# Codeuser0717/CVAE-GAN

Measured on NVIDIA B200. Metric: train_samples_per_s, higher is better.
Workload: dtype f32

## Files before the change

cvae_gan_b200/csrc/api.cu:

```cuda
#include "engine.cuh"

namespace cvg {
const char* last_error();
int comm_unique_id(void* out128);
int comm_init(Engine& e, const void* id128, int rank, int world);
void comm_destroy(Engine& e);
}

using namespace cvg;

struct CvgHandle {
  Engine e;
};

#define H_OR_FAIL(h)                      \
  if (!(h)) {                             \
    cvg::set_error("null handle");        \
    return 1;                             \
  }


constexpr int FC_MAX_KC = 12;
template <int KC>
struct FcDispatch {
// ... 34 lines not shown
int cvg_abi_version(void) { return CVG_ABI_VERSION; }
int cvg_config_bytes(void) { return (int)sizeof(CvgConfig); }

int cvg_create(const CvgConfig* cfg, CvgHandle** out) {
  if (!cfg || !out) CVG_FAIL("cvg_create: null argument");
  *out = nullptr;
  int dev = 0;
  CVG_CUDA(cudaGetDevice(&dev));
  cudaDeviceProp prop;
  CVG_CUDA(cudaGetDeviceProperties(&prop, dev));
  if (prop.major != 10)
    CVG_FAIL(std::string("cvaegan_b200 runs on sm_100 (B200) only; device is sm_") + std::to_string(prop.major) +
             std::to_string(prop.minor) + " - there is no fallback path");
  if (cfg->feature_num < 1 || cfg->label_num < 1 || cfg->z_size < 4 || cfg->max_batch < 1)
    CVG_FAIL("cvg_create: bad dimensions");
  if (cfg->world_size < 1 || cfg->rank < 0 || cfg->rank >= cfg->world_size) CVG_FAIL("cvg_create: bad rank/world_size");
  CvgHandle* h = new CvgHandle();
  Engine& e = h->e;
  e.cfg = *cfg;
  e.F = cfg->feature_num;
  e.K = cfg->label_num;
  e.Kc = cfg->unconditional ? 0 : cfg->label_num;
  e.Z = cfg->z_size;
  e.world = cfg->world_size;
  e.rank = cfg->rank;
  e.num_sms = prop.multiProcessorCount;
  if (build_layouts(e) != 0) {
    delete h;
    return 1;
  }
  set_all_kernel_attributes();
  tc_set_kernel_attributes();
  {
    const char* off = getenv("CVG_DISABLE_TC");
    e.use_tc = tc_supported(e) && !(off && off[0] == '1');
    const char* tm = getenv("CVG_TRAIN_MODE");
    e.mk.enabled = mk_supported(e) && tm && !strcmp(tm, "mk");
    if (const char* hv = getenv("CVG_HOIST")) e.hoist = atoi(hv) != 0;
    const char* coop = getenv("CVG_MK_COOP");
    e.mk.coop = !(coop && coop[0] == '0');
    const char* ab = getenv("CVG_MK_ALLBAR");
    e.mk.allbar = ab && ab[0] == '1';
  }
  if (cudaGetLastError() != cudaSuccess) {
    cvg::set_error("cudaFuncSetAttribute failed");
    delete h;
    return 1;
  }
  {
    SideStreams& ms = h->e.ms;
    const char* off = getenv("CVG_STREAMS");
    ms.on = !(off && off[0] == '0');
    bool ok = true;
    for (int i = 0; i < 2 && ok; ++i) ok = cudaStreamCreateWithFlags(&ms.s[i], cudaStreamNonBlocking) == cudaSuccess;
    for (int i = 0; i < SIDE_EVENTS && ok; ++i) ok = cudaEventCreateWithFlags(&ms.ev[i], cudaEventDisableTiming) == cudaSuccess;
    for (int i = 0; i < 4 && ok; ++i) ok = cudaEventCreateWithFlags(&ms.layer[i], cudaEventDisableTiming) == cudaSuccess;
    if (!ok) {
      cvg::set_error("creating the side streams failed");
      cvg_destroy(h);
      return 1;
    }
  }
  *out = h;
  return 0;
}

void cvg_destroy(CvgHandle* h) {
  if (!h) return;
  for (int i = 0; i < 2; ++i)
    if (h->e.ms.s[i]) cudaStreamDestroy(h->e.ms.s[i]);
  for (int i = 0; i < SIDE_EVENTS; ++i)
    if (h->e.ms.ev[i]) cudaEventDestroy(h->e.ms.ev[i]);
  for (int i = 0; i < 4; ++i)
    if (h->e.ms.layer[i]) cudaEventDestroy(h->e.ms.layer[i]);
  nvl_destroy(h->e);
  comm_destroy(h->e);
  mk_destroy(h->e);
  delete h;
}

int cvg_net_sizes(const CvgHandle* h, int net, int64_t* n_param_floats, int64_t* n_state_floats) {
  H_OR_FAIL(h);
  if (net < 0 || net >= CVG_NUM_NETS) CVG_FAIL("bad net id");
  if (n_param_floats) *n_param_floats = h->e.lay[net].n_param;
  if (n_state_floats) *n_state_floats = h->e.lay[net].n_state;
  return 0;
}

int cvg_tensor_table(const CvgHandle* h, int net, CvgTensorDesc* out, int32_t capacity, int32_t* count) {
  H_OR_FAIL(h);
  if (net < 0 || net >= CVG_NUM_NETS) CVG_FAIL("bad net id");
  const auto& t = h->e.lay[net].table;
  if (count) *count = (int32_t)t.size();
  if (out) {
    if (capacity < (int32_t)t.size()) CVG_FAIL("tensor table capacity too small");
    for (size_t i = 0; i < t.size(); ++i) out[i] = t[i];
  }
  return 0;
}

int64_t cvg_workspace_bytes(const CvgHandle* h) { return h ? workspace_bytes(h->e) : -1; }

int cvg_bind_net(CvgHandle* h, int net, float* params, float* grads, float* adam_m, float* adam_v, float* state) {
  H_OR_FAIL(h);
  if (net < 0 || net >= CVG_NUM_NETS) CVG_FAIL("bad net id");
  if (!params || !grads || !adam_m || !adam_v) CVG_FAIL("cvg_bind_net: null buffer");
  if (h->e.lay[net].n_state > 0 && !state) CVG_FAIL("cvg_bind_net: this network needs a state buffer");
  if ((((uintptr_t)params | (uintptr_t)grads | (uintptr_t)adam_m | (uintptr_t)adam_v | (uintptr_t)state) & 15) != 0)
    CVG_FAIL("cvg_bind_net: buffers must be 16-byte aligned");
  NetBuffers& b = h->e.buf[net];
  b.params = params; b.grads = grads; b.m = adam_m; b.v = adam_v; b.state = state;
  return 0;
}

int cvg_bind_workspace(CvgHandle* h, void* workspace, int64_t bytes, void* stream) {
  H_OR_FAIL(h);
  if (!workspace) CVG_FAIL("null workspace");
  CVG_TRY(carve_workspace(h->e, workspace, bytes));
  if (mk_supported(h->e)) CVG_TRY(mk_alloc_slots(h->e));
  CVG_CUDA(cudaMemsetAsync(workspace, 0, (size_t)bytes, (cudaStream_t)stream));
  return 0;
}
// ... 262 lines not shown
int cvg_debug_tc_counters(CvgHandle* h, long long* dev_counters) {
  H_OR_FAIL(h);
  h->e.tc_dbg = dev_counters;
  return 0;
}

int cvg_profile_enable(CvgHandle* h, int enable) {
  H_OR_FAIL(h);
  Engine& e = h->e;
  for (auto& r : e.prof_recs) {
    cudaEventDestroy(r.a);
    cudaEventDestroy(r.b);
  }
  e.prof_recs.clear();
  e.prof = enable != 0;
  return 0;
}

int cvg_profile_read(CvgHandle* h, int kernel_class, int64_t* launches, double* flops, double* ms) {
  H_OR_FAIL(h);
  if (!launches || !flops || !ms) CVG_FAIL("cvg_profile_read: null argument");
  Engine& e = h->e;
  *launches = 0;
  *flops = 0.0;
  *ms = 0.0;
  for (auto& r : e.prof_recs) {
    if (r.cls != kernel_class) continue;
    CVG_CUDA(cudaEventSynchronize(r.b));
    float t = 0.f;
    CVG_CUDA(cudaEventElapsedTime(&t, r.a, r.b));
    *launches += 1;
    *flops += r.flops;
    *ms += (double)t;
  }
  return 0;
}

int64_t cvg_launch_count(const CvgHandle* h) { return h ? h->e.launches : -1; }

int cvg_debug_set(CvgHandle* h, const char* key, int value) {
  H_OR_FAIL(h);
  if (!key) CVG_FAIL("null key");
  Engine& e = h->e;
  const std::string k(key);
  if (k == "train_mode") {
    if (value && !mk_supported(e)) CVG_FAIL("cvg_debug_set: the step-program kernel does not cover these layer widths");
    e.mk.enabled = value != 0;
  } else if (k == "mk_max_ops") e.mk.max_ops = value;
  else if (k == "mk_allbar") e.mk.allbar = value != 0;
  else if (k == "mk_coop") e.mk.coop = value != 0;
  else if (k == "hoist") e.hoist = value != 0;
  else if (k == "streams") e.ms.on = value != 0;
  else if (k == "chain") e.chain = value != 0;
  else if (k == "fuse_stats") e.nvl.fuse = value != 0;
  else CVG_FAIL("cvg_debug_set: unknown key");
  return 0;
}

int cvg_debug_get(const CvgHandle* h, const char* key, int* value) {
  H_OR_FAIL(h);
  if (!key || !value) CVG_FAIL("null argument");
  const Engine& e = h->e;
  const std::string k(key);
  if (k == "train_mode") *value = e.mk.enabled ? 1 : 0;
  else if (k == "mk_last_nops") *value = e.mk.last_nops;
  else if (k == "mk_supported") *value = mk_supported(e) ? 1 : 0;
  else CVG_FAIL("cvg_debug_get: unknown key");
  return 0;
}

int cvg_debug_mk_cycles(CvgHandle* h, long long* out, int capacity, int* count) {
  H_OR_FAIL(h);
  Engine& e = h->e;
  if (!e.ws_base) CVG_FAIL("workspace not bound");
  const int n = e.mk.last_nops < capacity ? e.mk.last_nops : capacity;
  if (count) *count = n;
  if (out && n > 0) CVG_CUDA(cudaMemcpy(out, e.ws.mk_dbg, sizeof(long long) * n, cudaMemcpyDeviceToHost));
  if (out && capacity >= 2048 + 64 && n <= 1024) {
    CVG_CUDA(cudaMemcpy(out + 1024, e.ws.mk_dbg + 1024, sizeof(long long) * n, cudaMemcpyDeviceToHost));
    if (capacity >= 4096)
      for (int i = 0; i < n && i < (int)e.mk.last_kinds.size(); ++i) out[3072 + i] = e.mk.last_kinds[i];
  }
  if (out && capacity >= 2048 + 64) CVG_CUDA(cudaMemcpy(out + 2048, e.ws.mk_dbg + 2048, sizeof(long long) * 64, cudaMemcpyDeviceToHost));
  return 0;
}

}
```

cvae_gan_b200/csrc/engine.cuh:

```cuda
#pragma once
#include "common.cuh"
#include "gemm.cuh"
#include "misc_kernels.cuh"
#include "comm_nvl.cuh"

typedef struct ncclComm* ncclComm_t;

namespace cvg {

constexpr int HOIST_MAX = 16;
constexpr int STAT_C = 1024;

constexpr int DET_MAX_PASS = 4;

struct Workspace {
  int ld = 0;
  int rows_cap = 0;
  float* xT = nullptr;
  float* z = nullptr;
  uint8_t* d_m1 = nullptr;
  uint8_t* d_m2 = nullptr;
  uint8_t* c_m1 = nullptr;
  uint8_t* c_m2 = nullptr;
  float *g_h[3] = {nullptr, nullptr, nullptr};
  float* g_out = nullptr;
  float* hz = nullptr;
  float* hh[3] = {nullptr, nullptr, nullptr};
  float* hout = nullptr;
  double* hfst = nullptr;
  float *g_dy[3] = {nullptr, nullptr, nullptr};
  float* g_dout = nullptr;
  float *e_h[3] = {nullptr, nullptr, nullptr};
  float* e_ml = nullptr;
  float *e_dy[3] = {nullptr, nullptr, nullptr};
  float* e_dml = nullptr;
  float *d_a[3] = {nullptr, nullptr, nullptr};
  float* d_s = nullptr;
  float *d_g[3] = {nullptr, nullptr, nullptr};
  float* c_a1 = nullptr;
  float* c_h2 = nullptr;
  float* c_a2 = nullptr;
  float* c_rs = nullptr;
  float* c_a3 = nullptr;
  float* c_logit = nullptr;
  float* c_dlogit = nullptr;
  float *c_g[3] = {nullptr, nullptr, nullptr};
  float* dx = nullptr;
  float* sn_sigma = nullptr;
  float* sn_inv_sigma = nullptr;
  float* sn_u = nullptr;
  float* sn_v = nullptr;
  long long sn_snap = 0;
  float* sn_G = nullptr;
  double* acc = nullptr;
  size_t acc_bytes = 0;
  double* loss = nullptr;
  double* g_fst = nullptr;
  double* g_bst = nullptr;
  double* e_fst = nullptr;
  double* e_bst = nullptr;
  unsigned long long* gen_count = nullptr;
  StepCtl* ctl = nullptr;
  float* x_stage = nullptr;
  float* tc_w = nullptr;
  float* tc_c = nullptr;
  float* dw_scratch = nullptr;
  long long dw_scratch_floats = 0;
  unsigned long long* det_acc[3] = {};
  unsigned* det_cnt[3] = {};
  long long det_acc_n = 0;
  int det_cnt_n = 0;
  unsigned int* mk_bar = nullptr;
  float* z_eps = nullptr;
  float* mk_wprep = nullptr;
  long long mk_wprep_floats = 0;
  long long* mk_dbg = nullptr;
};

struct MkSlot {
  void* dev = nullptr;
  void* host = nullptr;
  size_t bytes = 0;
  unsigned long long hash = 0;
  cudaEvent_t ev = nullptr;
  bool in_graph = false;
  unsigned long long last_use = 0;
};
struct MkPrepSlot {
  const float* W = nullptr;
  int ldw = 0, wcol0 = 0, wt = 0, R = 0, N = 0, net = -1;
  long long off = 0;
  bool fresh = false;
};
struct MkPendingRed {
  unsigned char bytes[160];
  int items;
};
struct MkState {
  bool enabled = true;
  bool coop = true;
  bool allbar = false;
  int max_ops = -1;
  bool recording = false;
  bool par_next = false;
  std::vector<unsigned char> ops;
  int nops = 0;
  int phase_items = 0;
  long long scratch_off = 0;
  int n_exchanges = 0;
  int adam_inc[4] = {0, 0, 0, 0};
  unsigned long long dcounter = 0;
  std::vector<MkPendingRed> pending_red;
  std::vector<MkPrepSlot> prep;
  long long prep_off = 0;
  bool prep_open = false;
  const float* src_rows = nullptr;
  long long src_n = 0, src_Bg = 0, src_off = 0;
  std::vector<MkSlot> slots;
  unsigned long long clock = 0;
  int last_nops = 0;
  std::vector<int> last_kinds;
};

struct ProfRec {
  cudaEvent_t a, b;
  int cls;
  double flops;
};

constexpr int SIDE_EVENTS = 32;
struct SideStreams {
  bool on = false;
  cudaStream_t s[2] = {nullptr, nullptr};
  cudaEvent_t ev[SIDE_EVENTS] = {};
  cudaEvent_t layer[4] = {};
  unsigned next = 0;
  bool dirty[2] = {false, false};
};

struct Engine {
  bool prof = false;
  std::vector<ProfRec> prof_recs;
  CvgConfig cfg{};
  int F = 0, K = 0, Z = 0;
  int Kc = 0;
  int eh[3]{}, gh[3]{}, dh[3]{}, ch[3]{};
  NetLayout lay[4];
  NetBuffers buf[4];
  Workspace ws;
  void* ws_base = nullptr;
  int64_t ws_bytes = 0;
  int64_t launches = 0;
  const float* hoist_x = nullptr;
  SideStreams ms;
  bool in_visit = false;
  unsigned long long step_dcounter = 0;
  int hoist = 1;
  bool chain = true;
  ncclComm_t comm = nullptr;
  int world = 1, rank = 0;
  NvlState nvl;
  int num_sms = 148;
  long long* tc_dbg = nullptr;
  bool use_tc = true;
  MkState mk;

  float* P(int net, int64_t off) const { return buf[net].params + off; }
  float* G(int net, int64_t off) const { return buf[net].grads + off; }
  float* S(int net, int64_t off) const { return buf[net].state + off; }
};

struct CvgHandleImpl {
  Engine e;
};

int build_layouts(Engine& e);
int64_t workspace_bytes(const Engine& e);
int carve_workspace(Engine& e, void* base, int64_t bytes);

struct StepRng {
  bool set = true;
  uint64_t seed = 0, counter = 0, off = 0;
  float lambda_class = 0.f;
  bool lambda_nonzero = true;
};
int step_d(Engine& e, const float* x_real, int label, int B, const CvgNoise* noise, const StepRng& rng, int flags,
           float* loss_out, cudaStream_t st);
int step_c(Engine& e, const float* x_real, int label, int B, const CvgNoise* noise, const StepRng& rng, int flags,
           float* loss_out, cudaStream_t st);
int step_g(Engine& e, const float* x_real, int label, int B, const CvgNoise* noise, const StepRng& rng, int flags,
           float* loss_out, cudaStream_t st);
int visit(Engine& e, int label, int B, int64_t B_global, const float* class_rows, int64_t n_rows, const float* x_batches,
          int d_loop, int c_loop, int g_loop, int flags, float* loss_out, cudaStream_t st);
void set_all_kernel_attributes();
struct AdamOverride {
  float lr, beta1, beta2, eps;
};
int run_adam(Engine& e, int net_mask, cudaStream_t st, const AdamOverride* ov = nullptr, bool steps_advanced = false);
int step_classifier(Engine& e, const float* x, const long long* labels, int B, const CvgNoise* noise, const StepRng& rng,
                    const AdamOverride& ov, int flags, float* loss_out, cudaStream_t st);
int nvl_local_handle(Engine& e, void* out64);
int nvl_attach(Engine& e, const void* handles);
void nvl_destroy(Engine& e);
int comm_all_reduce_f32(Engine& e, float* p, int64_t n, cudaStream_t st, int channel = 0);
int comm_all_reduce_f64(Engine& e, double* p, int64_t n, cudaStream_t st);
int comm_all_reduce_stats(Engine& e, double* p, int npass, int C, cudaStream_t st);

bool mk_supported(const Engine& e);
void mk_set_kernel_attributes();
void mk_destroy(Engine& e);
int mk_alloc_slots(Engine& e);
// ... 50 lines not shown
```

cvae_gan_b200/csrc/layout.cu:

```cuda
#include "engine.cuh"

namespace cvg {

static thread_local std::string g_err;
void set_error(const std::string& msg) { g_err = msg; }
const char* last_error() { return g_err.c_str(); }

static int64_t pad4(int64_t n) { return (n + 3) & ~(int64_t)3; }

struct Builder {
  NetLayout& L;
  int64_t po = 0, so = 0;
  explicit Builder(NetLayout& l) : L(l) {}
  int64_t add(const std::string& key, int kind, int64_t d0, int64_t d1) {
    CvgTensorDesc t;
    memset(&t, 0, sizeof(t));
    snprintf(t.key, sizeof(t.key), "%s", key.c_str());
    t.kind = kind;
    t.ndim = d1 > 0 ? 2 : 1;
    t.shape[0] = d0;
    t.shape[1] = d1 > 0 ? d1 : 0;
    const int64_t n = d0 * (d1 > 0 ? d1 : 1);
    int64_t& o = kind == 0 ? po : so;
    t.offset = o;
// ... 176 lines not shown
  w.c_a3 = c.take<float>(2 * e.ch[2] * ld);
  w.c_logit = c.take<float>(2 * K * ld);
  w.c_dlogit = c.take<float>(2 * K * ld);
  w.dx = c.take<float>(F * ld);
  w.sn_sigma = c.take<float>(8);
  w.sn_inv_sigma = c.take<float>(8);
  long long snap = 0;
  for (int i = 0; i < 4; ++i) {
    const LinearP& p = e.lay[CVG_NET_DISCRIMINATOR].lin[i];
    snap += pad4(p.out > p.in ? p.out : p.in);
  }
  w.sn_snap = snap;
  w.sn_u = c.take<float>(2 * snap);
  w.sn_v = c.take<float>(2 * snap);
  w.sn_G = c.take<float>(2 * e.lay[CVG_NET_DISCRIMINATOR].n_param);
  const size_t n_acc = 16 + (size_t)(3 * 2 + 3 * 2 + 3 + 3) * 2 * STAT_C;
  w.acc = c.take<double>(n_acc);
  w.acc_bytes = n_acc * sizeof(double);
  if (w.acc) {
    w.loss = w.acc;
    w.g_fst = w.acc + 16;
    w.g_bst = w.g_fst + (size_t)3 * 2 * 2 * STAT_C;
    w.e_fst = w.g_bst + (size_t)3 * 2 * 2 * STAT_C;
    w.e_bst = w.e_fst + (size_t)3 * 2 * STAT_C;
  }
  w.gen_count = c.take<unsigned long long>(4);
  w.ctl = c.take<StepCtl>(1);
  w.x_stage = c.take<float>((size_t)rows * F);
  w.tc_w = c.take<float>((size_t)tc_prep_floats(e));
  w.tc_c = c.take<float>((size_t)tc_const_floats());
  {
    long long per = 0;
    for (int net = 0; net < 4; ++net) {
      long long t = 0;
      for (int i = 0; i < e.lay[net].nlin; ++i) {
        const LinearP& p = e.lay[net].lin[i];
        t += (long long)p.out * (((p.in + 15) & ~15) + 1);
      }
      per += t * (net == CVG_NET_GENERATOR || net == CVG_NET_DISCRIMINATOR ? 2 : 1);
    }
    w.dw_scratch_floats = 32 * per;
  }
  w.dw_scratch = c.take<float>((size_t)w.dw_scratch_floats);
  {
    int tiles = 1, cmax = 1;
    for (int net = 0; net < 4; ++net)
      for (int i = 0; i < e.lay[net].nlin; ++i) {
        const LinearP& p = e.lay[net].lin[i];
        tiles = std::max(tiles, ((p.in + 63) / 64) * ((p.out + 63) / 64));
        cmax = std::max(cmax, std::max(p.in, p.out));
      }
    w.det_acc_n = std::max((long long)tiles * DET_MAX_PASS * DW_PART, 2LL * cmax);
    w.det_cnt_n = tiles;
    for (int i = 0; i < 3; ++i) {
      w.det_acc[i] = c.take<unsigned long long>((size_t)w.det_acc_n);
      w.det_cnt[i] = c.take<unsigned>((size_t)w.det_cnt_n);
    }
  }
  {
    long long chunks = 0;
    for (int net = 0; net < 4; ++net)
      for (int i = 0; i < e.lay[net].nlin; ++i) {
        const LinearP& p = e.lay[net].lin[i];
        chunks += (long long)((p.out + 127) / 128) * ((p.in + 31) / 32) + (long long)((p.in + 127) / 128) * ((p.out + 31) / 32);
      }
    w.mk_wprep_floats = chunks * 8192;
  }
  w.mk_wprep = c.take<float>((size_t)w.mk_wprep_floats);
  w.mk_bar = c.take<unsigned int>(64);
  w.z_eps = c.take<float>((size_t)Z * ld);
  w.mk_dbg = c.take<long long>(2048 + 64);
  w.hz = c.take<float>((size_t)HOIST_MAX * Z * ld);
  for (int i = 0; i < 3; ++i) w.hh[i] = c.take<float>((size_t)HOIST_MAX * e.gh[i] * ld);
  w.hout = c.take<float>((size_t)HOIST_MAX * F * ld);
  w.hfst = c.take<double>((size_t)3 * HOIST_MAX * 2 * STAT_C);
  return c.off + 256;
}

int64_t workspace_bytes(const Engine& e) {
  Workspace tmp;
  return (int64_t)carve(e, tmp, nullptr);
}

int carve_workspace(Engine& e, void* base, int64_t bytes) {
  if ((int64_t)workspace_bytes(e) > bytes) CVG_FAIL("workspace too small");
  if (((uintptr_t)base & 255) != 0) CVG_FAIL("workspace must be 256-byte aligned");
  carve(e, e.ws, base);
  e.ws_base = base;
  e.ws_bytes = bytes;
  return 0;
}

}
```

cvae_gan_b200/csrc/train.cu:

```cuda
#include <dlfcn.h>
#include <math.h>

#include "chain.cuh"
#include "engine.cuh"
#include "mega.cuh"

namespace cvg {

#define CVG_PAR(e) do { (e).mk.par_next = true; } while (0)

struct Id128 {
  char b[128];
};
struct NcclApi {
  int (*GetUniqueId)(void*) = nullptr;
  int (*CommInitRank)(ncclComm_t*, int, Id128, int) = nullptr;
  int (*AllReduce)(const void*, void*, size_t, int, int, ncclComm_t, cudaStream_t) = nullptr;
  int (*CommDestroy)(ncclComm_t) = nullptr;
  const char* (*GetErrorString)(int) = nullptr;
  bool ok = false;
};
static NcclApi g_nccl;

static int load_nccl() {
// ... 170 lines not shown
  cudaEventRecord(r.a, st);
  e.prof_recs.push_back(r);
}
static void prof_end(Engine& e, cudaStream_t st) {
  if (!e.prof) return;
  cudaEventRecord(e.prof_recs.back().b, st);
}

static const NvlDev* take_pending(Engine& e, Operand& o) {
  if (!e.nvl.n_pending || (o.kind != OP_BN_ACT && o.kind != OP_BN_BWD)) return nullptr;
  for (int i = 0; i < e.nvl.n_pending; ++i) {
    const NvlPending pd = e.nvl.pending[i];
    int which = 0;
    if (pd.stats == o.bn.fstats + (long long)pd.pass0 * o.bn.sf) which = 1;
    if (o.kind == OP_BN_BWD && pd.stats == o.bn.bstats + (long long)pd.pass0 * o.bn.sb) which = 2;
    if (!which) continue;
    o.bn.poll = which | (pd.npass << 4) | (pd.pass0 << 12) | (e.nvl.via_lead ? 1 << 20 : 0);
    e.nvl.pending[i] = e.nvl.pending[--e.nvl.n_pending];
    return e.nvl.dev_d[pd.channel];
  }
  return nullptr;
}

int launch_mn(Engine& e, bool wt, const GemmArgs& g_in, cudaStream_t st) {
  GemmArgs g = g_in;
  if (!e.mk.recording)
    if (const NvlDev* ch = take_pending(e, g.a)) g.nvl = ch;
  const int zp = g.only_pass >= 0 ? 1 : g.npass;
  if (e.mk.recording) {
    const int nmt = (g.N + 127) / 128;
    int Nt = 64;
    if ((long long)((g.M + 63) / 64) * nmt * zp > 3 * e.num_sms / 2) Nt = 128;
    if (const char* f = getenv("CVG_MK_NT")) { if (atoi(f) == 128 && g.M > 64) Nt = 128; if (atoi(f) == 64) Nt = 64; }
    const int items = zp * nmt * ((g.M + Nt - 1) / Nt);
    const bool par = e.mk.par_next;
    const float* wp = nullptr;
    bool prepped_now = false;
    CVG_TRY(mk_weight_operand(e, g, wt, &wp, &prepped_now));
    e.mk.par_next = par && !prepped_now;
    return mk_push(e, mk::K_MN, &g, GEMM_ARGS_OP_BYTES, items, wt ? 1 : 0, Nt, 0, 0, &wp, sizeof(wp));
  }
  dim3 grid((g.M + TBM - 1) / TBM, (g.N + TBN - 1) / TBN, zp);
  const size_t smem = gemm_mn_smem(g);
  prof_begin(e, wt ? 0 : 1, 2.0 * g.M * (double)g.N * g.R * zp, st);
  const cudaError_t err = dispatch_mn(wt, g, grid, smem, st);
  prof_end(e, st);
  if (err != cudaSuccess)
    CVG_FAIL(std::string("gemm_mn launch (a.kind ") + std::to_string(g.a.kind) + ", ekind " + std::to_string(g.ekind) +
             "): " + cudaGetErrorString(err));
  e.launches++;
  return 0;
}

static int det_slot(const Engine& e, cudaStream_t st) { return st == e.ms.s[0] ? 1 : st == e.ms.s[1] ? 2 : 0; }

int launch_dw(Engine& e, const DwArgs& g0, cudaStream_t st) {
  if (e.mk.recording) return mk_push_dw(e, g0);
  DwArgs g = g0;
  const int kt = (g.K + 63) / 64, nt = (g.N + 63) / 64;
  const int target = 2 * e.num_sms;
  int nsplit = (target + kt * nt * g.npass - 1) / (kt * nt * g.npass);
  const int max_split = (g.M + DW_MC - 1) / DW_MC;
  if (nsplit > max_split) nsplit = max_split;
  if (nsplit < 1) nsplit = 1;
  int rows = (g.M + nsplit - 1) / nsplit;
  rows = ((rows + DW_MC - 1) / DW_MC) * DW_MC;
  nsplit = (g.M + rows - 1) / rows;
  g.rows_per_cta = rows;
  if (const NvlDev* ch = take_pending(e, g.p)) g.nvl = ch;
  if (const NvlDev* ch = take_pending(e, g.q)) g.nvl = ch;
  dim3 grid(kt, nt, g.npass * nsplit);
  if ((long long)kt * nt * g.npass * DW_PART > e.ws.det_acc_n || kt * nt > e.ws.det_cnt_n)
    CVG_FAIL("internal: weight-gradient launch exceeds the deterministic-reduction slots");
  const int slot = det_slot(e, st);
  prof_begin(e, 2, 2.0 * g.M * (double)g.N * g.K * g.npass, st);
  const cudaError_t err = dispatch_dw(g, nsplit, e.ws.det_acc[slot], e.ws.det_cnt[slot], grid, gemm_dw_smem(g), st);
  prof_end(e, st);
  if (err != cudaSuccess)
    CVG_FAIL(std::string("gemm_dw launch (p.kind ") + std::to_string(g.p.kind) + ", q.kind " + std::to_string(g.q.kind) +
             "): " + cudaGetErrorString(err));
  e.launches++;
  return 0;
}

static const LinearP& lin(const Engine& e, int net, int l) { return e.lay[net].lin[l]; }

static const float* label_column(const Engine& e, int net, const LinearP& p, int in_width, int label) {
  return e.Kc > 0 ? e.P(net, p.w) + in_width + label : nullptr;
}
static int label_col_index(const Engine& e, int in_width, int label) { return e.Kc > 0 ? in_width + label : -1; }

static double* fst_of(const Engine& e, int net, int l) {
  return net == CVG_NET_GENERATOR ? e.ws.g_fst + (size_t)l * 2 * 2 * STAT_C : e.ws.e_fst + (size_t)l * 2 * STAT_C;
}
static double* bst_of(const Engine& e, int net, int l) {
  return net == CVG_NET_GENERATOR ? e.ws.g_bst + (size_t)l * 2 * 2 * STAT_C : e.ws.e_bst + (size_t)l * 2 * STAT_C;
}

static BnRef bn_ref(const Engine& e, int net, int l, bool eval, bool update) {
  const LinearP& p = lin(e, net, l);
  BnRef b;
  b.fstats = fst_of(e, net, l);
  b.sf = 2 * STAT_C;
  b.bstats = bst_of(e, net, l);
  b.sb = 2 * STAT_C;
  b.gamma = e.P(net, p.gamma);
  b.beta = e.P(net, p.beta);
// ... 13 lines not shown
  g.Bg = Bg_bn;
  g.bn_eps = e.cfg.bn_eps;
  g.momentum = e.cfg.bn_momentum;
  g.slope = e.cfg.lrelu_slope;
  return g;
}

static DwArgs base_dw(const Engine& e, int M, float Bg_bn, int npass) {
  DwArgs g;
  g.M = M;
  g.ld = e.ws.ld;
  g.npass = npass;
  g.Bg = Bg_bn;
  g.bn_eps = e.cfg.bn_eps;
  g.slope = e.cfg.lrelu_slope;
  return g;
}

static int sync_stats(Engine& e, double* p, int npass, int C, bool local_bn, cudaStream_t st) {
  if (e.world <= 1 || local_bn) return 0;
  return comm_all_reduce_stats(e, p, npass, C, st);
}

static bool fold_stats(const Engine& e, bool local_bn) {
  return e.world > 1 && !local_bn && e.nvl.on && e.nvl.fuse && e.nvl.dev_d[0] && !e.mk.recording;
}
static int launch_mn_stats(Engine& e, bool wt, GemmArgs& g, int npass_sync, bool local_bn, cudaStream_t st, int channel = 0) {
  const bool fold = fold_stats(e, local_bn);
  if (!fold && channel != 0 && e.world > 1 && !local_bn) CVG_FAIL("internal: an exchange launch on a side stream");
  if (fold) { g.push = 1; g.nvl = e.nvl.dev_d[channel]; }
  CVG_TRY(launch_mn(e, wt, g, st));
  if (!fold) return sync_stats(e, g.ostats, npass_sync, g.N, local_bn, st);
  if (e.nvl.n_pending >= 8) CVG_FAIL("internal: too many folded exchanges in flight");
  const int p0 = g.only_pass > 0 ? g.only_pass : 0;
  e.nvl.pending[e.nvl.n_pending++] = NvlPending{g.ostats + (long long)p0 * g.sostats, g.only_pass >= 0 ? 1 : g.npass, p0, channel};
  return 0;
}

static cudaStream_t fork_to(Engine& e, int i, cudaStream_t st) {
  if (!e.ms.on || e.mk.recording) return st;
  cudaEvent_t ev = e.ms.ev[e.ms.next++ % SIDE_EVENTS];
  cudaEventRecord(ev, st);
  cudaStreamWaitEvent(e.ms.s[i], ev, 0);
  e.ms.dirty[i] = true;
  return e.ms.s[i];
}
static void wait_for(Engine& e, cudaStream_t waiter, cudaStream_t signaller) {
  if (waiter == signaller) return;
  cudaEvent_t ev = e.ms.ev[e.ms.next++ % SIDE_EVENTS];
  cudaEventRecord(ev, signaller);
  cudaStreamWaitEvent(waiter, ev, 0);
}
static void join_sides(Engine& e, cudaStream_t st, int only = -1) {
  for (int i = 0; i < 2; ++i) {
    if (!e.ms.dirty[i] || (only >= 0 && only != i)) continue;
    cudaEvent_t ev = e.ms.ev[e.ms.next++ % SIDE_EVENTS];
    cudaEventRecord(ev, e.ms.s[i]);
    cudaStreamWaitEvent(st, ev, 0);
    e.ms.dirty[i] = false;
  }
}

static int launch_fill(Engine& e, FillArgs& a, cudaStream_t st) {
  if (a.njobs == 0) return 0;
  if (e.mk.recording) return mk_push(e, mk::K_FILL, &a, sizeof(a), a.njobs * mk::FILL_VB);
  long long mx = 0;
  for (int i = 0; i < a.njobs; ++i) {
    long long t = (long long)a.job[i].npass * ((a.job[i].nfeat + 3) / 4) * a.M;
    if (t > mx) mx = t;
  }
  int blocks = (int)((mx + 255) / 256);
  if (blocks > 4 * e.num_sms) blocks = 4 * e.num_sms;
  if (blocks < 1) blocks = 1;
  fill_noise_kernel<<<dim3(blocks, a.njobs), 256, 0, st>>>(a);
  CVG_LAUNCH_CHECK();
  return 0;
}

static void add_job(FillArgs& a, void* out, const void* inj, int kind, int nfeat, int npass, int stream) {
  FillJob& j = a.job[a.njobs++];
  j.out = out;
  j.injected = inj;
  j.kind = kind;
  j.nfeat = nfeat;
  j.npass = npass;
  j.stream = stream;
  j.cstep = 0;
}

static int emit_zero(Engine& e, void* p, size_t bytes, cudaStream_t st) {
  if (e.mk.recording) {
    mk::ZeroArgs a;
    a.p = p; a.bytes = (long long)bytes;
    const int items = (int)((bytes / 16 + mk::THREADS * 8 - 1) / (mk::THREADS * 8));
    return mk_push(e, mk::K_ZERO, &a, sizeof(a), items < 1 ? 1 : items);
  }
  CVG_CUDA(cudaMemsetAsync(p, 0, bytes, st));
  return 0;
}

static int stage_x(Engine& e, const float* x_real, int M, cudaStream_t st) {
  if (e.mk.recording) {
    const MkState& src = e.mk;
    mk::StageArgs a;
    memset(&a, 0, sizeof(a));
    a.src = src.src_rows ? src.src_rows : x_real;
    a.n_rows = src.src_rows ? src.src_n : 0;
// ... 436 lines not shown
    g.W = e.P(net, p.w);
    g.ldw = p.in;
    if (l == 0) {
      g.ekind = EP_STORE;
      g.Y = w.dx;
      g.accumulate = dx_accumulate ? 1 : 0;
    } else {
      g.ekind = EP_DACT;
      g.act = ACT_RELU;
      g.sprev = (long long)p.in * ld;
      g.sY = (long long)p.in * ld;
      g.Y = w.c_g[l - 1];
      if (l == 3) g.prev = w.c_a3;
      if (l == 2) { g.prev = w.c_a2; g.mask = w.c_m2; g.smask = (long long)p.in * ld; g.keep_inv = keep_inv; }
      if (l == 1) { g.prev = w.c_a1; g.mask = w.c_m1; g.smask = (long long)p.in * ld; g.keep_inv = keep_inv; }
    }
    if (want_dw) CVG_PAR(e);
    CVG_TRY(launch_mn(e, false, g, st));
    if (l == 2) {
      const LinearP& p1 = lin(e, net, 1);
      LnBwdArgs a;
      a.M = M; a.ld = w.ld; a.C = p1.out; a.npass = npass;
      a.dn = w.c_g[1]; a.sdn = (long long)p1.out * ld;
      a.h = w.c_h2; a.sh = (long long)p1.out * ld;
      a.rs = w.c_rs; a.srs = 2 * (long long)ld;
      a.g = e.P(net, p1.gamma);
      a.dg = want_dw ? e.G(net, p1.gamma) : nullptr;
      a.db = want_dw ? e.G(net, p1.beta) : nullptr;
      if (e.mk.recording) {
        CVG_TRY(mk_push(e, mk::K_LN_BWD, &a, sizeof(a), npass * ((M + 31) / 32)));
      } else {
        const int slot = det_slot(e, st);
        if (2LL * a.C > e.ws.det_acc_n) CVG_FAIL("internal: LayerNorm backward exceeds the deterministic-reduction slots");
        launch_ln_bwd(a, e.ws.det_acc[slot], e.ws.det_cnt[slot], st);
        CVG_LAUNCH_CHECK();
      }
    }
  }
  return 0;
}

struct BnNetBwd {
  int net, npass;
  float* const* h;
  float* const* dy;
  const float* top_dy;
  long long s_top;
  Operand first_in;
  int first_K;
  int label_col;
  bool want_first_dx;
};

static int bwd_bn_net(Engine& e, const BnNetBwd& b, int M, float Bg_bn, float kl_coef, bool local_bn, cudaStream_t st) {
  const Workspace& w = e.ws;
  const size_t ld = w.ld;
  const int net = b.net;
  for (int l = 3; l >= 0; --l) {
    const LinearP& p = lin(e, net, l);
    Operand dy;
    if (l == 3) {
      dy.kind = OP_PLAIN; dy.rows = p.out; dy.p = b.top_dy; dy.sp = b.s_top;
    } else {
      dy.kind = OP_BN_BWD; dy.rows = p.out;
      dy.p = b.dy[l]; dy.sp = (long long)p.out * ld;
      dy.h = b.h[l]; dy.sh = (long long)p.out * ld;
      dy.bn = bn_ref(e, net, l, false, false);
    }
    if (l > 0) {
      const LinearP& pp = lin(e, net, l - 1);
      GemmArgs g = base_args(e, M, Bg_bn, b.npass);
      g.R = p.out;
      g.N = p.in;
      g.a = dy;
      g.W = e.P(net, p.w);
      g.ldw = p.in;
      g.ekind = EP_DBN;
      g.prev = b.h[l - 1];
      g.sprev = (long long)pp.out * ld;
      g.prev_bn = bn_ref(e, net, l - 1, false, false);
      g.Y = b.dy[l - 1];
      g.sY = (long long)pp.out * ld;
      g.ostats = bst_of(e, net, l - 1);
      g.sostats = 2 * STAT_C;
      CVG_TRY(launch_mn_stats(e, false, g, b.npass, local_bn, st));
    } else if (b.want_first_dx) {
      GemmArgs g = base_args(e, M, Bg_bn, b.npass);
      g.only_pass = 0;
      g.R = p.out;
      g.N = e.Z;
      g.a = dy;
      g.W = e.P(net, p.w);
      g.ldw = p.in;
      g.ekind = EP_REPARAM_BWD;
      g.mu = w.e_ml;
      g.lv = w.e_ml + (size_t)e.Z * ld;
      g.eps = e.mk.recording ? w.z_eps : w.z;
      g.kl_coef = kl_coef;
      g.Y = w.e_dml;
      CVG_TRY(launch_mn(e, false, g, st));
    }
    if (l > 0 || b.want_first_dx) CVG_PAR(e);
    DwArgs d = base_dw(e, M, Bg_bn, b.npass);
    d.N = p.out;
    d.p = dy;
    if (l == 0) {
      d.K = b.first_K;
      d.q = b.first_in;
      d.label_col = b.label_col;
    } else {
      d.K = p.in;
      d.q.kind = OP_BN_ACT;
      d.q.rows = p.in;
      d.q.p = b.h[l - 1];
      d.q.sp = (long long)p.in * ld;
      d.q.bn = bn_ref(e, net, l - 1, false, false);
    }
    d.dW = e.G(net, p.w);
    d.sdW = 0;
    d.ldw = p.in;
    d.db = e.G(net, p.b);
    if (l < 3) {
      d.dgamma = e.G(net, p.gamma);
      d.dbeta = e.G(net, p.beta);
      d.add_affine = (e.world <= 1 || local_bn || e.rank == 0) ? 1 : 0;
    }
    CVG_TRY(launch_dw(e, d, fork_to(e, 0, st)));
  }
  return 0;
}

static float net_lr(const Engine& e, int net) {
  if (net == CVG_NET_DISCRIMINATOR) return e.cfg.d_lr;
  if (net == CVG_NET_CLASSIFIER) return e.cfg.c_lr;
  return e.cfg.g_lr;
}

int run_adam(Engine& e, int net_mask, cudaStream_t st, const AdamOverride* ov, bool steps_advanced) {
  AdamArgs a;
  a.nseg = 0;
  a.b1 = ov ? ov->beta1 : e.cfg.adam_beta1;
  a.b2 = ov ? ov->beta2 : e.cfg.adam_beta2;
  a.eps = ov ? ov->eps : e.cfg.adam_eps;
  a.clear_grad = 1;
  long long nmax = 0;
  for (int net = 0; net < 4; ++net) {
    if (!(net_mask & (1 << net))) continue;
    if (a.nseg == 2) CVG_FAIL("cvg_adam: at most two networks per call");
    AdamSeg& s = a.seg[a.nseg++];
    s.p = e.buf[net].params; s.g = e.buf[net].grads; s.m = e.buf[net].m; s.v = e.buf[net].v;
    s.n = e.lay[net].n_param;
    s.lr = ov ? ov->lr : net_lr(e, net);
    s.t_prev = &e.ws.ctl->adam_t[net];
    if (s.n > nmax) nmax = s.n;
  }
  if (a.nseg == 0) return 0;
  if (e.mk.recording) {
    mk::AdamOp op;
    op.a = a;
    op.t_off[0] = op.t_off[1] = 0;
    int si = 0;
    for (int net = 0; net < 4; ++net)
      if (net_mask & (1 << net)) { op.t_off[si++] = e.mk.adam_inc[net]; e.mk.adam_inc[net]++; }
    mk_weights_updated(e, net_mask);
    return mk_push(e, mk::K_ADAM, &op, sizeof(op), a.nseg * mk::ADAM_VB);
  }
  int blocks = (int)((nmax + 255) / 256);
  if (blocks > 2 * e.num_sms) blocks = 2 * e.num_sms;
  a.t_add = steps_advanced ? 0 : 1;
  adam_kernel<<<dim3(blocks, a.nseg), 256, 0, st>>>(a);
  CVG_LAUNCH_CHECK();
  if (!steps_advanced) {
    ctl_bump_kernel<<<1, 32, 0, st>>>(e.ws.ctl, 0ull, net_mask);
    CVG_LAUNCH_CHECK();
  }
  return 0;
}

static int finish_step(Engine& e, int net_mask, int kind, int M, int flags, float* loss_out, cudaStream_t st,
                       const AdamOverride* ov = nullptr) {
// ... 412 lines not shown
  gb.want_first_dx = true;
  CVG_TRY(bwd_bn_net(e, gb, B, Bg_bn, e.cfg.lambda_kl / Bg, local_bn, st));
  BnNetBwd eb;
  eb.net = E; eb.npass = 1;
  eb.h = w.e_h; eb.dy = w.e_dy;
  eb.top_dy = w.e_dml; eb.s_top = 0;
  eb.first_in.kind = OP_PLAIN; eb.first_in.rows = e.F; eb.first_in.p = w.xT;
  eb.first_K = e.F;
  eb.label_col = label_col_index(e, e.F, label);
  eb.want_first_dx = false;
  CVG_TRY(bwd_bn_net(e, eb, B, Bg_bn, 0.f, local_bn, st));
  return finish_step(e, (1 << E) | (1 << G), 2, B, flags, loss_out, st);
}

int step_g(Engine& e, const float* x_real, int label, int B, const CvgNoise* nz, const StepRng& rng, int flags,
           float* loss_out, cudaStream_t st) {
  if (flags & CVG_STEP_PRIOR_ONLY) return step_g_prior(e, label, B, nz, rng, flags, loss_out, st);
  if (flags & CVG_STEP_CVAE) return step_g_cvae(e, x_real, label, B, nz, rng, flags, loss_out, st);
  CVG_TRY(check_step(e, B));
  ProgramScope prog(e);
  CVG_TRY(begin_step(e, rng, true, st));
  const Workspace& w = e.ws;
  const size_t ld = w.ld;
  const bool local_bn = flags & CVG_STEP_LOCAL_BN;
  const float Bg = (float)B * (float)e.world;
  const float Bg_bn = local_bn ? (float)B : Bg;
  const int E = CVG_NET_ENCODER, G = CVG_NET_GENERATOR;
  if (rng.set) CVG_PAR(e);
  CVG_TRY(emit_zero(e, w.acc, w.acc_bytes, st));
  CVG_TRY(prep_net(e, E, true, true, false));
  CVG_TRY(prep_net(e, G, true, true, true));
  CVG_TRY(prep_net(e, CVG_NET_DISCRIMINATOR, true, true, true));
  CVG_TRY(prep_net(e, CVG_NET_CLASSIFIER, true, rng.lambda_nonzero, true));
  FillArgs f;
  fill_args(e, f, rng, B);
  add_job(f, e.mk.recording ? w.z_eps : w.z, nz ? nz->eps : nullptr, 0, e.Z, 1, RS_EPS);
  add_job(f, w.z + (size_t)e.Z * ld, nz ? nz->z : nullptr, 0, e.Z, 1, RS_Z);
  add_job(f, w.d_m1, nz ? nz->d_mask1 : nullptr, 1, e.dh[0], 1, RS_DMASK1);
  add_job(f, w.d_m2, nz ? nz->d_mask2 : nullptr, 1, e.dh[1], 1, RS_DMASK2);
  add_job(f, w.c_m1, nz ? nz->c_mask1 : nullptr, 1, e.ch[0], 1, RS_CMASK1);
  add_job(f, w.c_m2, nz ? nz->c_mask2 : nullptr, 1, e.ch[1], 1, RS_CMASK2);
  CVG_PAR(e);
  CVG_TRY(launch_fill(e, f, st));
  const float* x_fake = w.g_out + (size_t)e.F * ld;
  CeArgs c;
  c.M = B; c.ld = w.ld; c.K = e.K; c.npass = 1; c.label = label;
  c.logits = w.c_logit; c.sl = (long long)e.K * ld;
  c.dlogits = w.c_dlogit; c.sd = (long long)e.K * ld;
  c.coef = 1.0f / Bg;
  c.ctl = w.ctl;
  c.loss = w.loss + L_CE0;
  const float seedv[2] = {-e.cfg.lambda_adv / Bg, 0.f};
  const bool three = !e.mk.recording && e.ms.on && (e.world <= 1 || local_bn || fold_stats(e, local_bn));
  join_sides(e, st);
  if (three) {
    const cudaStream_t sA = fork_to(e, 0, st), sB = fork_to(e, 1, st);
    CVG_TRY(launch_sn(e, 1, true, sA));
    CVG_TRY(stage_x(e, x_real, B, sB));
    wait_for(e, st, sB);
    GenSplit prior;
    prior.only_pass = 1; prior.channel = 1; prior.rec = e.ms.layer;
    CVG_TRY(fwd_generator(e, 2, true, false, label, B, Bg_bn, local_bn, sB, nullptr, &prior));
    wait_for(e, sB, sA);
    if (rng.lambda_nonzero) {
      wait_for(e, sA, sB);
      CVG_TRY(fwd_classifier(e, x_fake, 0, 1, true, B, sA));
      CVG_TRY(emit_ce(e, c, B, 1, sA));
    }
    CVG_TRY(fwd_critic(e, x_fake, 0, 1, label, B, w.loss + L_DFAKE, sB));
    CVG_TRY(bwd_critic(e, x_fake, 0, 1, label, B, seedv, false, true, sB));
    if (rng.lambda_nonzero) CVG_TRY(bwd_classifier(e, x_fake, 0, 1, B, false, true, true, sA, sB));
    CVG_TRY(fwd_encoder(e, true, label, B, Bg_bn, local_bn, st));
    GenSplit enc;
    enc.only_pass = 0; enc.channel = 0; enc.wait = e.ms.layer;
    CVG_TRY(fwd_generator(e, 2, true, true, label, B, Bg_bn, local_bn, st, nullptr, &enc));
    join_sides(e, st);
  } else {
  CVG_PAR(e);
  CVG_TRY(stage_x(e, x_real, B, fork_to(e, 1, st)));

  CVG_PAR(e);
  CVG_TRY(launch_sn(e, 1, true, fork_to(e, 0, st)));
  join_sides(e, st, 1);
  CVG_TRY(fwd_encoder(e, true, label, B, Bg_bn, local_bn, st));
  if (e.mk.recording) {
    mk::ReparamArgs ra;
    ra.mu = w.e_ml; ra.lv = w.e_ml + (size_t)e.Z * ld; ra.eps = w.z_eps; ra.out = w.z; ra.M = B; ra.ld = w.ld; ra.Z = e.Z;
    CVG_TRY(mk_push(e, mk::K_REPARAM, &ra, sizeof(ra), (int)(((long long)e.Z * ld + mk::THREADS - 1) / mk::THREADS)));
  }
  CVG_TRY(fwd_generator(e, 2, true, true, label, B, Bg_bn, local_bn, st));
  join_sides(e, st);
  const cudaStream_t sc = rng.lambda_nonzero ? fork_to(e, 1, st) : st;
  CVG_TRY(fwd_critic(e, x_fake, 0, 1, label, B, w.loss + L_DFAKE, st));
  CVG_TRY(fwd_classifier(e, x_fake, 0, 1, true, B, sc));
  CVG_TRY(emit_ce(e, c, B, 1, sc));
  CVG_TRY(bwd_critic(e, x_fake, 0, 1, label, B, seedv, false, true, st));
  if (rng.lambda_nonzero) CVG_TRY(bwd_classifier(e, x_fake, 0, 1, B, false, true, true, sc, st));
  join_sides(e, st);
  }

  SeedArgs s;
  s.M = B; s.ld = w.ld; s.F = e.F;
  s.out = w.g_out; s.sout = (long long)e.F * ld;
  s.x = w.xT; s.dx = w.dx;
  s.dpre = w.g_dout; s.sdpre = (long long)e.F * ld;
  s.coef_recon = e.cfg.lambda_recon / (Bg * (float)e.F);
  s.recon_acc = w.loss + L_RECON;
  if (e.mk.recording) {
    CVG_TRY(mk_push(e, mk::K_SEED, &s, sizeof(s), 2 * (int)(((long long)e.F * ld + mk::THREADS - 1) / mk::THREADS)));
  } else {
    g_seed_kernel<<<dim3((unsigned)((e.F * ld + 255) / 256), 2), 256, 0, st>>>(s);
    CVG_LAUNCH_CHECK();
  }

  const LinearP& g0 = lin(e, G, 0);
  BnNetBwd gb;
  gb.net = G; gb.npass = 2;
  gb.h = w.g_h; gb.dy = w.g_dy;
  gb.top_dy = w.g_dout; gb.s_top = (long long)e.F * ld;
  gb.first_in.kind = e.mk.recording ? OP_PLAIN : OP_REPARAM; gb.first_in.rows = e.Z;
  gb.first_in.p = w.z; gb.first_in.sp = (long long)e.Z * ld;
  gb.first_in.mu = w.e_ml; gb.first_in.lv = w.e_ml + (size_t)e.Z * ld; gb.first_in.eps = w.z;
  gb.first_in.reparam_pass = 0;
  gb.first_K = e.Z;
  gb.label_col = label_col_index(e, e.Z, label);
  gb.want_first_dx = true;
  (void)g0;
  CVG_TRY(bwd_bn_net(e, gb, B, Bg_bn, e.cfg.lambda_kl / Bg, local_bn, st));

  BnNetBwd eb;
  eb.net = E; eb.npass = 1;
  eb.h = w.e_h; eb.dy = w.e_dy;
  eb.top_dy = w.e_dml; eb.s_top = 0;
  eb.first_in.kind = OP_PLAIN; eb.first_in.rows = e.F; eb.first_in.p = w.xT;
  eb.first_K = e.F;
  eb.label_col = label_col_index(e, e.F, label);
  eb.want_first_dx = false;
  CVG_TRY(bwd_bn_net(e, eb, B, Bg_bn, 0.f, local_bn, st));

  CVG_TRY(finish_step(e, (1 << E) | (1 << G), 2, B, flags, loss_out, st));
  return prog.finish(st);
}

static int hoist_generator(Engine& e, int nh, int label, int B, int flags, cudaStream_t st) {
  const Workspace& w = e.ws;
  const bool local_bn = flags & CVG_STEP_LOCAL_BN;
  const float Bg_bn = local_bn ? (float)B : (float)B * (float)e.world;
  StepRng rng;
  rng.set = false;
  rng.off = 1;
  if (e.mk.recording) e.mk.par_next = false;
  join_sides(e, st);
  CVG_TRY(emit_zero(e, w.hfst, sizeof(double) * 3 * HOIST_MAX * 2 * STAT_C, st));
  CVG_TRY(prep_net(e, CVG_NET_GENERATOR, true, false, false));
  FillArgs f;
  fill_args(e, f, rng, B);
  add_job(f, w.hz, nullptr, 0, e.Z, nh, RS_Z);
  f.job[0].cstep = 2;
  CVG_PAR(e);
  CVG_TRY(launch_fill(e, f, st));
  GenBufs b;
  b.z = w.hz; b.out = w.hout;
  for (int l = 0; l < 3; ++l) { b.h[l] = w.hh[l]; b.fst[l] = w.hfst + (size_t)l * HOIST_MAX * 2 * STAT_C; }
  return fwd_generator(e, nh, true, false, label, B, Bg_bn, local_bn, st, &b);
}

int visit(Engine& e, int label, int B, int64_t B_global, const float* class_rows, int64_t n_rows, const float* x_batches,
          int d_loop, int c_loop, int g_loop, int flags, float* loss_out, cudaStream_t st) {
  CVG_TRY(check_step(e, B));
  if (!x_batches && (!class_rows || n_rows < 1)) CVG_FAIL("cvg_visit: need class_rows or x_batches");
  if (B_global != (int64_t)B * e.world) CVG_FAIL("cvg_visit: B_global must be B_local * world_size");
  ProgramScope prog(e);
  struct InVisit { Engine& e; explicit InVisit(Engine& en) : e(en) { e.in_visit = true; } ~InVisit() { e.in_visit = false; } } in_visit(e);
  const int nh = e.hoist ? (d_loop + c_loop < HOIST_MAX ? d_loop + c_loop : HOIST_MAX) : 0;
  if (nh > 0) CVG_TRY(hoist_generator(e, nh, label, B, flags, st));
  int i = 0;
  for (int kind = 0; kind < 3; ++kind) {
    const int reps = kind == 0 ? d_loop : (kind == 1 ? c_loop : g_loop);
    for (int r = 0; r < reps; ++r, ++i) {
      e.hoist_x = (kind < 2 && i < nh) ? e.ws.hout + (size_t)i * e.F * e.ws.ld : nullptr;
      const float* x = nullptr;
      const bool no_batch = kind == 2 && (flags & CVG_STEP_PRIOR_ONLY);
      if (no_batch) {
        x = nullptr;
      } else if (x_batches) {
        x = x_batches + (size_t)i * B * e.F;
      } else if (e.mk.recording) {
        e.mk.src_rows = class_rows; e.mk.src_n = n_rows; e.mk.src_Bg = B_global; e.mk.src_off = (long long)e.rank * B;
        x = class_rows;
      } else {
        sample_rows_kernel<<<(B + 127) / 128, 128, 0, fork_to(e, 1, st)>>>(class_rows, n_rows, B_global, (long long)e.rank * B,
// ... 44 lines not shown
```

Measured before the change: 12.89 million.

## Split generator backward passes across streams and add third side stream for encoder dW

Adds a third side stream and, when multi-stream mode is on with a single device or local BN, splits the generator backward by pass: pass 0 dX runs on the main stream and pass 1 dX on a side stream, while dW runs on another side stream. The seed kernel is likewise split per pass. Encoder dW launches go to the new third stream so they overlap the encoder dX chain, and the join before the seed is skipped. The aim is more concurrency among the small GEMMs of a latency-bound step. The cost is more event waits and extra deterministic-accumulator slots, and the hand-written dependency ordering could race if any edge is missing.

```diff
diff --git a/cvae_gan_b200/csrc/api.cu b/cvae_gan_b200/csrc/api.cu
--- a/cvae_gan_b200/csrc/api.cu
+++ b/cvae_gan_b200/csrc/api.cu
@@ -110,7 +110,7 @@
     const char* off = getenv("CVG_STREAMS");
     ms.on = !(off && off[0] == '0');
     bool ok = true;
-    for (int i = 0; i < 2 && ok; ++i) ok = cudaStreamCreateWithFlags(&ms.s[i], cudaStreamNonBlocking) == cudaSuccess;
+    for (int i = 0; i < SIDE_STREAMS && ok; ++i) ok = cudaStreamCreateWithFlags(&ms.s[i], cudaStreamNonBlocking) == cudaSuccess;
     for (int i = 0; i < SIDE_EVENTS && ok; ++i) ok = cudaEventCreateWithFlags(&ms.ev[i], cudaEventDisableTiming) == cudaSuccess;
     for (int i = 0; i < 4 && ok; ++i) ok = cudaEventCreateWithFlags(&ms.layer[i], cudaEventDisableTiming) == cudaSuccess;
     if (!ok) {
@@ -125,7 +125,7 @@
 
 void cvg_destroy(CvgHandle* h) {
   if (!h) return;
-  for (int i = 0; i < 2; ++i)
+  for (int i = 0; i < SIDE_STREAMS; ++i)
     if (h->e.ms.s[i]) cudaStreamDestroy(h->e.ms.s[i]);
   for (int i = 0; i < SIDE_EVENTS; ++i)
     if (h->e.ms.ev[i]) cudaEventDestroy(h->e.ms.ev[i]);
@@ -494,6 +494,7 @@
   else if (k == "hoist") e.hoist = value != 0;
   else if (k == "streams") e.ms.on = value != 0;
   else if (k == "chain") e.chain = value != 0;
+  else if (k == "eg_split") e.eg_split = value != 0;
   else if (k == "fuse_stats") e.nvl.fuse = value != 0;
   else CVG_FAIL("cvg_debug_set: unknown key");
   return 0;
diff --git a/cvae_gan_b200/csrc/engine.cuh b/cvae_gan_b200/csrc/engine.cuh
--- a/cvae_gan_b200/csrc/engine.cuh
+++ b/cvae_gan_b200/csrc/engine.cuh
@@ -12,6 +12,7 @@
 constexpr int STAT_C = 1024;
 
 constexpr int DET_MAX_PASS = 4;
+constexpr int SIDE_STREAMS = 3;
 
 struct Workspace {
   int ld = 0;
@@ -66,8 +67,8 @@
   float* tc_c = nullptr;
   float* dw_scratch = nullptr;
   long long dw_scratch_floats = 0;
-  unsigned long long* det_acc[3] = {};
-  unsigned* det_cnt[3] = {};
+  unsigned long long* det_acc[SIDE_STREAMS + 1] = {};
+  unsigned* det_cnt[SIDE_STREAMS + 1] = {};
   long long det_acc_n = 0;
   int det_cnt_n = 0;
   unsigned int* mk_bar = nullptr;
@@ -131,11 +132,11 @@
 constexpr int SIDE_EVENTS = 32;
 struct SideStreams {
   bool on = false;
-  cudaStream_t s[2] = {nullptr, nullptr};
+  cudaStream_t s[SIDE_STREAMS] = {};
   cudaEvent_t ev[SIDE_EVENTS] = {};
   cudaEvent_t layer[4] = {};
   unsigned next = 0;
-  bool dirty[2] = {false, false};
+  bool dirty[SIDE_STREAMS] = {};
 };
 
 struct Engine {
@@ -157,6 +158,7 @@
   unsigned long long step_dcounter = 0;
   int hoist = 1;
   bool chain = true;
+  bool eg_split = true;
   ncclComm_t comm = nullptr;
   int world = 1, rank = 0;
   NvlState nvl;
diff --git a/cvae_gan_b200/csrc/layout.cu b/cvae_gan_b200/csrc/layout.cu
--- a/cvae_gan_b200/csrc/layout.cu
+++ b/cvae_gan_b200/csrc/layout.cu
@@ -252,7 +252,7 @@
       }
     w.det_acc_n = std::max((long long)tiles * DET_MAX_PASS * DW_PART, 2LL * cmax);
     w.det_cnt_n = tiles;
-    for (int i = 0; i < 3; ++i) {
+    for (int i = 0; i < SIDE_STREAMS + 1; ++i) {
       w.det_acc[i] = c.take<unsigned long long>((size_t)w.det_acc_n);
       w.det_cnt[i] = c.take<unsigned>((size_t)w.det_cnt_n);
     }
diff --git a/cvae_gan_b200/csrc/train.cu b/cvae_gan_b200/csrc/train.cu
--- a/cvae_gan_b200/csrc/train.cu
+++ b/cvae_gan_b200/csrc/train.cu
@@ -246,7 +246,11 @@
   return 0;
 }
 
-static int det_slot(const Engine& e, cudaStream_t st) { return st == e.ms.s[0] ? 1 : st == e.ms.s[1] ? 2 : 0; }
+static int det_slot(const Engine& e, cudaStream_t st) {
+  for (int i = 0; i < SIDE_STREAMS; ++i)
+    if (st == e.ms.s[i]) return 1 + i;
+  return 0;
+}
 
 int launch_dw(Engine& e, const DwArgs& g0, cudaStream_t st) {
   if (e.mk.recording) return mk_push_dw(e, g0);
@@ -366,7 +370,7 @@
   cudaStreamWaitEvent(waiter, ev, 0);
 }
 static void join_sides(Engine& e, cudaStream_t st, int only = -1) {
-  for (int i = 0; i < 2; ++i) {
+  for (int i = 0; i < SIDE_STREAMS; ++i) {
     if (!e.ms.dirty[i] || (only >= 0 && only != i)) continue;
     cudaEvent_t ev = e.ms.ev[e.ms.next++ % SIDE_EVENTS];
     cudaEventRecord(ev, e.ms.s[i]);
@@ -909,80 +913,97 @@
   bool want_first_dx;
 };
 
-static int bwd_bn_net(Engine& e, const BnNetBwd& b, int M, float Bg_bn, float kl_coef, bool local_bn, cudaStream_t st) {
+static Operand bn_net_dy(const Engine& e, const BnNetBwd& b, int l) {
+  const LinearP& p = lin(e, b.net, l);
+  Operand dy;
+  if (l == 3) {
+    dy.kind = OP_PLAIN; dy.rows = p.out; dy.p = b.top_dy; dy.sp = b.s_top;
+  } else {
+    dy.kind = OP_BN_BWD; dy.rows = p.out;
+    dy.p = b.dy[l]; dy.sp = (long long)p.out * e.ws.ld;
+    dy.h = b.h[l]; dy.sh = (long long)p.out * e.ws.ld;
+    dy.bn = bn_ref(e, b.net, l, false, false);
+  }
+  return dy;
+}
+
+static int bwd_bn_dx(Engine& e, const BnNetBwd& b, int l, int M, float Bg_bn, float kl_coef, bool local_bn, cudaStream_t st,
+                     int only_pass = -1) {
   const Workspace& w = e.ws;
   const size_t ld = w.ld;
   const int net = b.net;
+  const LinearP& p = lin(e, net, l);
+  if (l > 0) {
+    const LinearP& pp = lin(e, net, l - 1);
+    GemmArgs g = base_args(e, M, Bg_bn, b.npass);
+    g.only_pass = only_pass;
+    g.R = p.out;
+    g.N = p.in;
+    g.a = bn_net_dy(e, b, l);
+    g.W = e.P(net, p.w);
+    g.ldw = p.in;
+    g.ekind = EP_DBN;
+    g.prev = b.h[l - 1];
+    g.sprev = (long long)pp.out * ld;
+    g.prev_bn = bn_ref(e, net, l - 1, false, false);
+    g.Y = b.dy[l - 1];
+    g.sY = (long long)pp.out * ld;
+    g.ostats = bst_of(e, net, l - 1);
+    g.sostats = 2 * STAT_C;
+    return launch_mn_stats(e, false, g, b.npass, local_bn, st);
+  }
+  if (!b.want_first_dx) return 0;
+  GemmArgs g = base_args(e, M, Bg_bn, b.npass);
+  g.only_pass = 0;
+  g.R = p.out;
+  g.N = e.Z;
+  g.a = bn_net_dy(e, b, l);
+  g.W = e.P(net, p.w);
+  g.ldw = p.in;
+  g.ekind = EP_REPARAM_BWD;
+  g.mu = w.e_ml;
+  g.lv = w.e_ml + (size_t)e.Z * ld;
+  g.eps = e.mk.recording ? w.z_eps : w.z;
+  g.kl_coef = kl_coef;
+  g.Y = w.e_dml;
+  return launch_mn(e, false, g, st);
+}
+
+static int bwd_bn_dw(Engine& e, const BnNetBwd& b, int l, int M, float Bg_bn, bool local_bn, cudaStream_t st) {
+  const int net = b.net;
+  const LinearP& p = lin(e, net, l);
+  DwArgs d = base_dw(e, M, Bg_bn, b.npass);
+  d.N = p.out;
+  d.p = bn_net_dy(e, b, l);
+  if (l == 0) {
+    d.K = b.first_K;
+    d.q = b.first_in;
+    d.label_col = b.label_col;
+  } else {
+    d.K = p.in;
+    d.q.kind = OP_BN_ACT;
+    d.q.rows = p.in;
+    d.q.p = b.h[l - 1];
+    d.q.sp = (long long)p.in * e.ws.ld;
+    d.q.bn = bn_ref(e, net, l - 1, false, false);
+  }
+  d.dW = e.G(net, p.w);
+  d.sdW = 0;
+  d.ldw = p.in;
+  d.db = e.G(net, p.b);
+  if (l < 3) {
+    d.dgamma = e.G(net, p.gamma);
+    d.dbeta = e.G(net, p.beta);
+    d.add_affine = (e.world <= 1 || local_bn || e.rank == 0) ? 1 : 0;
+  }
+  return launch_dw(e, d, st);
+}
+
+static int bwd_bn_net(Engine& e, const BnNetBwd& b, int M, float Bg_bn, float kl_coef, bool local_bn, cudaStream_t st) {
   for (int l = 3; l >= 0; --l) {
-    const LinearP& p = lin(e, net, l);
-    Operand dy;
-    if (l == 3) {
-      dy.kind = OP_PLAIN; dy.rows = p.out; dy.p = b.top_dy; dy.sp = b.s_top;
-    } else {
-      dy.kind = OP_BN_BWD; dy.rows = p.out;
-      dy.p = b.dy[l]; dy.sp = (long long)p.out * ld;
-      dy.h = b.h[l]; dy.sh = (long long)p.out * ld;
-      dy.bn = bn_ref(e, net, l, false, false);
-    }
-    if (l > 0) {
-      const LinearP& pp = lin(e, net, l - 1);
-      GemmArgs g = base_args(e, M, Bg_bn, b.npass);
-      g.R = p.out;
-      g.N = p.in;
-      g.a = dy;
-      g.W = e.P(net, p.w);
-      g.ldw = p.in;
-      g.ekind = EP_DBN;
-      g.prev = b.h[l - 1];
-      g.sprev = (long long)pp.out * ld;
-      g.prev_bn = bn_ref(e, net, l - 1, false, false);
-      g.Y = b.dy[l - 1];
-      g.sY = (long long)pp.out * ld;
-      g.ostats = bst_of(e, net, l - 1);
-      g.sostats = 2 * STAT_C;
-      CVG_TRY(launch_mn_stats(e, false, g, b.npass, local_bn, st));
-    } else if (b.want_first_dx) {
-      GemmArgs g = base_args(e, M, Bg_bn, b.npass);
-      g.only_pass = 0;
-      g.R = p.out;
-      g.N = e.Z;
-      g.a = dy;
-      g.W = e.P(net, p.w);
-      g.ldw = p.in;
-      g.ekind = EP_REPARAM_BWD;
-      g.mu = w.e_ml;
-      g.lv = w.e_ml + (size_t)e.Z * ld;
-      g.eps = e.mk.recording ? w.z_eps : w.z;
-      g.kl_coef = kl_coef;
-      g.Y = w.e_dml;
-      CVG_TRY(launch_mn(e, false, g, st));
-    }
+    CVG_TRY(bwd_bn_dx(e, b, l, M, Bg_bn, kl_coef, local_bn, st));
     if (l > 0 || b.want_first_dx) CVG_PAR(e);
-    DwArgs d = base_dw(e, M, Bg_bn, b.npass);
-    d.N = p.out;
-    d.p = dy;
-    if (l == 0) {
-      d.K = b.first_K;
-      d.q = b.first_in;
-      d.label_col = b.label_col;
-    } else {
-      d.K = p.in;
-      d.q.kind = OP_BN_ACT;
-      d.q.rows = p.in;
-      d.q.p = b.h[l - 1];
-      d.q.sp = (long long)p.in * ld;
-      d.q.bn = bn_ref(e, net, l - 1, false, false);
-    }
-    d.dW = e.G(net, p.w);
-    d.sdW = 0;
-    d.ldw = p.in;
-    d.db = e.G(net, p.b);
-    if (l < 3) {
-      d.dgamma = e.G(net, p.gamma);
-      d.dbeta = e.G(net, p.beta);
-      d.add_affine = (e.world <= 1 || local_bn || e.rank == 0) ? 1 : 0;
-    }
-    CVG_TRY(launch_dw(e, d, fork_to(e, 0, st)));
+    CVG_TRY(bwd_bn_dw(e, b, l, M, Bg_bn, local_bn, fork_to(e, 0, st)));
   }
   return 0;
 }
@@ -1501,6 +1522,7 @@
   c.loss = w.loss + L_CE0;
   const float seedv[2] = {-e.cfg.lambda_adv / Bg, 0.f};
   const bool three = !e.mk.recording && e.ms.on && (e.world <= 1 || local_bn || fold_stats(e, local_bn));
+  const bool split = three && e.eg_split && (e.world <= 1 || local_bn);
   join_sides(e, st);
   if (three) {
     const cudaStream_t sA = fork_to(e, 0, st), sB = fork_to(e, 1, st);
@@ -1523,7 +1545,7 @@
     GenSplit enc;
     enc.only_pass = 0; enc.channel = 0; enc.wait = e.ms.layer;
     CVG_TRY(fwd_generator(e, 2, true, true, label, B, Bg_bn, local_bn, st, nullptr, &enc));
-    join_sides(e, st);
+    if (!split) join_sides(e, st);
   } else {
   CVG_PAR(e);
   CVG_TRY(stage_x(e, x_real, B, fork_to(e, 1, st)));
@@ -1555,14 +1577,25 @@
   s.dpre = w.g_dout; s.sdpre = (long long)e.F * ld;
   s.coef_recon = e.cfg.lambda_recon / (Bg * (float)e.F);
   s.recon_acc = w.loss + L_RECON;
+  const unsigned seed_blocks = (unsigned)((e.F * ld + 255) / 256);
   if (e.mk.recording) {
     CVG_TRY(mk_push(e, mk::K_SEED, &s, sizeof(s), 2 * (int)(((long long)e.F * ld + mk::THREADS - 1) / mk::THREADS)));
+  } else if (split) {
+    const cudaStream_t sB = e.ms.s[1];
+    g_seed_kernel<<<dim3(seed_blocks, 1), 256, 0, st>>>(s);
+    CVG_LAUNCH_CHECK();
+    SeedArgs s1 = s;
+    s1.out += (size_t)e.F * ld;
+    s1.dpre += (size_t)e.F * ld;
+    s1.prior_only = 1;
+    if (rng.lambda_nonzero) wait_for(e, sB, e.ms.s[0]);
+    g_seed_kernel<<<dim3(seed_blocks, 1), 256, 0, sB>>>(s1);
+    CVG_LAUNCH_CHECK();
   } else {
-    g_seed_kernel<<<dim3((unsigned)((e.F * ld + 255) / 256), 2), 256, 0, st>>>(s);
+    g_seed_kernel<<<dim3(seed_blocks, 2), 256, 0, st>>>(s);
     CVG_LAUNCH_CHECK();
   }
 
-  const LinearP& g0 = lin(e, G, 0);
   BnNetBwd gb;
   gb.net = G; gb.npass = 2;
   gb.h = w.g_h; gb.dy = w.g_dy;
@@ -1574,8 +1607,7 @@
   gb.first_K = e.Z;
   gb.label_col = label_col_index(e, e.Z, label);
   gb.want_first_dx = true;
-  (void)g0;
-  CVG_TRY(bwd_bn_net(e, gb, B, Bg_bn, e.cfg.lambda_kl / Bg, local_bn, st));
+  const float kl_coef = e.cfg.lambda_kl / Bg;
 
   BnNetBwd eb;
   eb.net = E; eb.npass = 1;
@@ -1585,7 +1617,25 @@
   eb.first_K = e.F;
   eb.label_col = label_col_index(e, e.F, label);
   eb.want_first_dx = false;
-  CVG_TRY(bwd_bn_net(e, eb, B, Bg_bn, 0.f, local_bn, st));
+
+  if (split) {
+    const cudaStream_t sA = e.ms.s[0], sB = e.ms.s[1];
+    for (int l = 3; l >= 0; --l) {
+      wait_for(e, sA, st);
+      wait_for(e, sA, sB);
+      CVG_TRY(bwd_bn_dx(e, gb, l, B, Bg_bn, kl_coef, local_bn, st, 0));
+      if (l > 0) CVG_TRY(bwd_bn_dx(e, gb, l, B, Bg_bn, kl_coef, local_bn, sB, 1));
+      CVG_TRY(bwd_bn_dw(e, gb, l, B, Bg_bn, local_bn, sA));
+    }
+    for (int l = 3; l >= 0; --l) {
+      const cudaStream_t sw = fork_to(e, 2, st);
+      CVG_TRY(bwd_bn_dx(e, eb, l, B, Bg_bn, 0.f, local_bn, st));
+      CVG_TRY(bwd_bn_dw(e, eb, l, B, Bg_bn, local_bn, sw));
+    }
+  } else {
+    CVG_TRY(bwd_bn_net(e, gb, B, Bg_bn, kl_coef, local_bn, st));
+    CVG_TRY(bwd_bn_net(e, eb, B, Bg_bn, 0.f, local_bn, st));
+  }
 
   CVG_TRY(finish_step(e, (1 << E) | (1 << G), 2, B, flags, loss_out, st));
   return prog.finish(st);
```

Measured after the change: 13.78 million (median of 6 runs). 6.9% higher.
